# saninsteinn/django-assistant-bot

Measured on AMD Instinct MI355X. Metric: RAG queries/sec + p50 end-to-end latency, bge-base + Llama-3-8B, 1/2/4/8 MI355X, higher is better.
Workload: dtype bf16; 1 GPU; model=bge-base-en + llama-3-8b, global_batch=128, seq_len=1090, parallelism=dp1, mode=batch, index_rows=1000000, index=single shard, local top-k (no collective), sampling=temperature=1.0 top_k=50 top_p=0.95 ignore_eos, graphs=True

## Files before the change

### django_assistant_bot_amd/csrc/bindings.cpp

```cpp
#include <hip/hip_runtime.h>
#include <pybind11/numpy.h>
#include <pybind11/pybind11.h>
#include <pybind11/stl.h>

#include <stdexcept>
#include <string>

#include "kernels/launchers.h"
#include "runtime/json_grammar.h"
#include "runtime/kv_manager.h"
#include "runtime/rag.h"
#include "runtime/tokenizer.h"
#include "runtime/trace.h"

namespace py = pybind11;
using u = uintptr_t;

#define VP(x) reinterpret_cast<void*>(x)
#define CVP(x) reinterpret_cast<const void*>(x)
#define ST(x) reinterpret_cast<hipStream_t>(x)

static void check(int err, const char* name) {
  if (err) throw std::runtime_error(std::string("dab kernel '") + name + "' failed: " + hipGetErrorString((hipError_t)err));
}
// ... 91 lines not shown
                                     (const int*)ctx_k, batch, max_sq, Hq, Hkv, D, causal, paged, scale, ST(s)),
                "flash_attention");
        });
  m.def("flash_attention_rope",
        [](u q, long qst, long qsh, u kc, u vc, u bt, int max_blocks, int bs, u out, long ost, long osh, u cu_q,
           u ctx_k, int batch, int max_sq, int Hq, int Hkv, int D, int causal, float scale, u rope_pos, u rope_cs,
           u s) {
          check(dab::flash_attention(CVP(q), qst, qsh, nullptr, nullptr, 0, 0, CVP(kc), CVP(vc), (const int*)bt,
                                     max_blocks, bs, VP(out), ost, osh, (const int*)cu_q, nullptr, (const int*)ctx_k,
                                     batch, max_sq, Hq, Hkv, D, causal, 1, scale, ST(s), (const int*)rope_pos,
                                     CVP(rope_cs)),
                "flash_attention_rope");
        });
  m.def("create_cu_masked_stream", [](std::vector<uint32_t> mask) {
    hipStream_t st = nullptr;
    check(hipExtStreamCreateWithCUMask(&st, (uint32_t)mask.size(), mask.data()), "hipExtStreamCreateWithCUMask");
    return reinterpret_cast<uintptr_t>(st);
  });
  m.def("destroy_stream", [](u s) { check(hipStreamDestroy(ST(s)), "hipStreamDestroy"); });
  m.def("paged_decode_attention", [](u q, u kc, u vc, u bt, int max_blocks, int bs, u ctx, u out, u po, u pm, u pl,
                                     u cnt, int batch, int Hq, int Hkv, int D, int part_size, int max_parts,
                                     float scale, u s, u order, u w0, long w0_bytes, u w1, long w1_bytes,
                                     int w_blocks) {
    dab::L3Warm warm{{(const char*)w0, (const char*)w1}, {w0_bytes, w1_bytes}, w_blocks};
    check(dab::paged_decode_attention(CVP(q), CVP(kc), CVP(vc), (const int*)bt, max_blocks, bs, (const int*)ctx, VP(out),
                                      (float*)po, (float*)pm, (float*)pl, (int*)cnt, batch, Hq, Hkv, D, part_size,
                                      max_parts, scale, ST(s), (const int*)order, &warm),
          "paged_decode_attention");
  }, py::arg("q"), py::arg("kc"), py::arg("vc"), py::arg("bt"), py::arg("max_blocks"), py::arg("bs"), py::arg("ctx"),
     py::arg("out"), py::arg("po"), py::arg("pm"), py::arg("pl"), py::arg("cnt"), py::arg("batch"), py::arg("Hq"),
     py::arg("Hkv"), py::arg("D"), py::arg("part_size"), py::arg("max_parts"), py::arg("scale"), py::arg("s"),
     py::arg("order") = 0, py::arg("w0") = 0, py::arg("w0_bytes") = 0, py::arg("w1") = 0, py::arg("w1_bytes") = 0,
     py::arg("w_blocks") = 0);
  m.def("rope_kv_write_fp8", [](u qkv, int ld, u positions, u cos_sin, u q_out, u k_data, u k_exp, u v_data, u v_exp,
                                u slots, int T, int Hq, int Hkv, int D, int block_size, u s, u slabs, int S,
                                long slab_stride, int slab_bf16) {
    check(dab::rope_kv_write_fp8(CVP(qkv), ld, (const int*)positions, CVP(cos_sin), VP(q_out), VP(k_data), VP(k_exp),
                                 VP(v_data), VP(v_exp), (const int64_t*)slots, T, Hq, Hkv, D, block_size, ST(s),
                                 CVP(slabs), S, slab_stride, slab_bf16),
          "rope_kv_write_fp8");
  }, py::arg("qkv"), py::arg("ld"), py::arg("positions"), py::arg("cos_sin"), py::arg("q_out"), py::arg("k_data"),
     py::arg("k_exp"), py::arg("v_data"), py::arg("v_exp"), py::arg("slots"), py::arg("T"), py::arg("Hq"),
     py::arg("Hkv"), py::arg("D"), py::arg("block_size"), py::arg("s"), py::arg("slabs") = 0, py::arg("S") = 0,
     py::arg("slab_stride") = 0, py::arg("slab_bf16") = 0);
  m.def("kv_fp8_dequant_blocks", [](u k_data, u k_exp, u v_data, u v_exp, u ids, int n, u k_out, u v_out, int Hkv,
                                    int block_size, int D, u s) {
    check(dab::kv_fp8_dequant_blocks(CVP(k_data), CVP(k_exp), CVP(v_data), CVP(v_exp), (const int*)ids, n, VP(k_out),
                                     VP(v_out), Hkv, block_size, D, ST(s)),
          "kv_fp8_dequant_blocks");
  });
  m.def("paged_decode_attention_fp8", [](u q, u k_data, u k_exp, u v_data, u v_exp, u bt, int max_blocks, int bs, u ctx,
                                         u out, u po, u pm, u pl, u cnt, int batch, int Hq, int Hkv, int D,
                                         int part_size, int max_parts, float scale, u s, u order) {
    check(dab::paged_decode_attention_fp8(CVP(q), CVP(k_data), CVP(k_exp), CVP(v_data), CVP(v_exp), (const int*)bt,
                                          max_blocks, bs, (const int*)ctx, VP(out), (float*)po, (float*)pm, (float*)pl,
                                          (int*)cnt, batch, Hq, Hkv, D, part_size, max_parts, scale, ST(s),
                                          (const int*)order),
          "paged_decode_attention_fp8");
  });
  m.def("gemm_bt", [](u A, long lda, u B, long ldb, u C, long ldc, u bias, u residual, long ldr, int M, int N, int K,
                      int epilogue, int out_f32, u row_group, u q_group, u allow, int allow_words, u s, int b_rows,
                      int b_group) {
    check(dab::gemm_bt(CVP(A), lda, CVP(B), ldb, VP(C), ldc, CVP(bias), CVP(residual), ldr, M, N, K, epilogue, out_f32,
                       (const int*)row_group, (const int*)q_group, (const uint32_t*)allow, allow_words, ST(s), b_rows,
                       b_group),
          "gemm_bt");
// ... 291 lines not shown
```

### django_assistant_bot_amd/csrc/kernels/attention.hip

```cpp
#include <cstdlib>

#include "common.h"
#include "launchers.h"

#include <type_traits>

#define DAB_ALWAYS_INLINE __attribute__((always_inline))

namespace dab {

constexpr float kNegInf = -__builtin_huge_valf();

template <int D>
__device__ __forceinline__ int swz(int r, int c) {
  constexpr int RB = D * 2;
  constexpr int CPR = D / 8;
  constexpr int RPB = (256 / RB) > 0 ? (256 / RB) : 1;
  return r * RB + 16 * (c ^ ((2 * (r / RPB)) & (CPR - 1)));
}

struct FlashParams {
  const bf16* q;
  long q_stride_tok, q_stride_head;
  const bf16* k;
// ... 1246 lines not shown
        for (int t = 0; t < NTD; ++t) o[t] = f32x4{0.f, 0.f, 0.f, 0.f};
        m_run = -1e30f;
        l_run = 0.f;
      }
    }
    if (n.it < 0) break;
    if (new_q) {
#pragma unroll
      for (int kk = 0; kk < NKK; ++kk) qf[kk] = qn[kk];
    }
    c = n;
  }
}


struct DecodeParams {
  const bf16* q;
  const bf16* k_cache;
  const bf16* v_cache;
  const int* block_tables;
  int max_blocks, block_size;
  const int* ctx_lens;
  bf16* out;
  float* part_o;
  float* part_m;
  float* part_l;
  int* counters;
  const int* order;
  int Hq, Hkv, part_size, max_parts;
  float scale_log2;
  L3Warm warm;
};

template <int D, bool KV_NT, bool DMA = false, int NSLOT = 1>
__global__ __launch_bounds__(256, NSLOT == 1 ? 2 : 1) void paged_decode_kernel(DecodeParams p, int total_items) {
  static_assert(NSLOT == 1 || (NSLOT == 2 && DMA), "two slots: DMA staging only");
  const int attn_blocks = gridDim.x - p.warm.blocks;
  if ((int)blockIdx.x >= attn_blocks) {
    l3_warm(p.warm, blockIdx.x - attn_blocks);
    return;
  }
  constexpr int KT = 32;
  constexpr int NKK = D / 32;
  constexpr int NTD = D / 16;
  constexpr int CPR = D / 8;
  constexpr int SUB_BYTES = KT * D * 2;
  constexpr int CH = KT * CPR / 64;
  constexpr int RED_BYTES = 4 * 16 * D * 4 + 2 * 4 * 16 * 4;
  constexpr int STAGE_BYTES = 4 * 2 * SUB_BYTES * NSLOT;
  constexpr int AREA_BYTES = STAGE_BYTES > RED_BYTES + 16 ? STAGE_BYTES : RED_BYTES + 16;
  __shared__ __attribute__((aligned(16))) char smem[AREA_BYTES];
  int* last_flag = reinterpret_cast<int*>(smem + RED_BYTES);

  const int G = p.Hq / p.Hkv;
  const int tid = threadIdx.x, lane = tid & 63, g = lane >> 4, li = lane & 15;
  const int w = __builtin_amdgcn_readfirstlane(tid >> 6);
  char* ks = smem + w * 2 * SUB_BYTES * NSLOT;
  char* vs = ks + SUB_BYTES;

  const int BH = total_items / p.max_parts;
  int maxc = 0;
  for (int i = lane; i < BH / p.Hkv; i += 64) maxc = max(maxc, p.ctx_lens[i]);
#pragma unroll
  for (int off = 32; off; off >>= 1) maxc = max(maxc, __shfl_xor(maxc, off));
  maxc = __builtin_amdgcn_readfirstlane(maxc);
  const int live_items = min(p.max_parts, (maxc + p.part_size - 1) / p.part_size) * BH;
  for (int item = blockIdx.x; item < live_items; item += attn_blocks) {
    const int part = item / BH;
    const int bh = item - part * BH;
    const int hk = bh % p.Hkv, b = p.order ? p.order[bh / p.Hkv] : bh / p.Hkv;
    const int ctx = p.ctx_lens[b];
    const int k_begin = part * p.part_size;
    if (k_begin >= ctx) continue;
    const int k_end = min(ctx, k_begin + p.part_size);

    bf16x8 qf[NKK];
    {
      const bool qv = li < G;
      const bf16* qrow = p.q + ((size_t)b * p.Hq + hk * G + (qv ? li : 0)) * D;
#pragma unroll
      for (int kk = 0; kk < NKK; ++kk) {
        bf16x8 z = {0, 0, 0, 0, 0, 0, 0, 0};
        qf[kk] = qv ? *reinterpret_cast<const bf16x8*>(qrow + 32 * kk + 8 * g) : z;
      }
    }

    u32x4 kA[CH], vA[CH], kB[CH], vB[CH];
    const int k_last = ((k_end - 1) / KT) * KT;
    auto load_sub = [&](u32x4(&kr)[CH], u32x4(&vr)[CH], int k0) {
      const int kc = min(k0, k_last);
      const int blk = p.block_tables[(size_t)b * p.max_blocks + kc / p.block_size];
      const size_t base = (((size_t)blk * p.Hkv + hk) * p.block_size + (kc % p.block_size)) * D;
      const int bytes = k0 > k_last ? 0 : min(KT, k_end - k0) * D * 2;
      const auto kd = __builtin_amdgcn_make_buffer_rsrc((void*)(p.k_cache + base), 0, bytes, 0x00020000);
      const auto vd = __builtin_amdgcn_make_buffer_rsrc((void*)(p.v_cache + base), 0, bytes, 0x00020000);
#pragma unroll
      for (int c = 0; c < CH; ++c) {
        kr[c] = __builtin_bit_cast(u32x4, __builtin_amdgcn_raw_buffer_load_b128(kd, lane * 16, c * 1024, KV_NT ? 2 : 0));
        vr[c] = __builtin_bit_cast(u32x4, __builtin_amdgcn_raw_buffer_load_b128(vd, lane * 16, c * 1024, KV_NT ? 2 : 0));
      }
    };
    auto stage = [&](const u32x4(&kr)[CH], const u32x4(&vr)[CH]) {
#pragma unroll
      for (int c = 0; c < CH; ++c) {
        const int idx = lane + c * 64;
        const int row = idx / CPR, ch = idx % CPR;
        *reinterpret_cast<u32x4*>(ks + swz<D>(row, ch)) = kr[c];
        *reinterpret_cast<u32x4*>(vs + swz<D>(row, ch)) = vr[c];
      }
    };

    f32x4 o[NTD];
#pragma unroll
    for (int t = 0; t < NTD; ++t) o[t] = f32x4{0.f, 0.f, 0.f, 0.f};
    float m_run = -1e30f, l_run = 0.f;

    auto compute = [&](const int k0) {
      __builtin_amdgcn_s_waitcnt(0xc07f);
// ... 36 lines not shown
      }
      l_run = l_run * alpha + ls;
      m_run = m_new;
      bf16x8 pb;
#pragma unroll
      for (int j = 0; j < 4; ++j) {
        pb[j] = (short)f2bf(s[0][j]);
        pb[j + 4] = (short)f2bf(s[1][j]);
      }
      const int qq = li >> 2, pp = li & 3;
#pragma unroll
      for (int t = 0; t < NTD; ++t) {
        o[t] *= alpha;
        const int ch = 2 * t + (pp >> 1);
        const int boff = 8 * (pp & 1);
        const bf16x4 lo = ds_read_tr16(vs + swz<D>(4 * g + qq, ch) + boff);
        const bf16x4 hi = ds_read_tr16(vs + swz<D>(16 + 4 * g + qq, ch) + boff);
        const bf16x8 a = {lo[0], lo[1], lo[2], lo[3], hi[0], hi[1], hi[2], hi[3]};
        o[t] = mfma16(a, pb, o[t]);
      }
      __builtin_amdgcn_s_waitcnt(0xc07f);
      __builtin_amdgcn_wave_barrier();
    };
    const int kw = k_begin + w * KT;
    if constexpr (DMA) {
      static_assert(D == 128, "DMA staging assumes 256-B rows (4 rows per 1 KB piece)");
      const int drow = lane >> 4;
      auto blk_at = [&](int k0) {
        return p.block_tables[(size_t)b * p.max_blocks + min(k0, k_last) / p.block_size];
      };
      auto dma = [&](int k0, int blk) {
        const int kc = min(k0, k_last);
        const size_t base = (((size_t)blk * p.Hkv + hk) * p.block_size + (kc % p.block_size)) * D;
        const int bytes = k0 > k_last ? 0 : min(KT, k_end - k0) * D * 2;
        const auto kd = __builtin_amdgcn_make_buffer_rsrc((void*)(p.k_cache + base), 0, bytes, 0x00020000);
        const auto vd = __builtin_amdgcn_make_buffer_rsrc((void*)(p.v_cache + base), 0, bytes, 0x00020000);
#pragma unroll
        for (int i = 0; i < KT / 4; ++i) {
          const int row = 4 * i + drow;
          const unsigned off = (unsigned)(row * 256 + 16 * ((lane & 15) ^ ((2 * row) & 15)));
          __builtin_amdgcn_raw_ptr_buffer_load_lds(kd, (__attribute__((address_space(3))) void*)(ks + i * 1024), 16, off,
                                                   0, 0, KV_NT ? 2 : 0);
          __builtin_amdgcn_raw_ptr_buffer_load_lds(vd, (__attribute__((address_space(3))) void*)(vs + i * 1024), 16, off,
                                                   0, 0, KV_NT ? 2 : 0);
        }
      };
      if constexpr (NSLOT == 2) {
        char* const slot0 = smem + w * 2 * SUB_BYTES * NSLOT;
        const int n_sub = kw < k_end ? (k_end - kw + 4 * KT - 1) / (4 * KT) : 0;
        const int myblk = lane < n_sub ? blk_at(kw + lane * 4 * KT) : 0;
        auto issue = [&](int i) {
          ks = slot0 + (i & 1) * 2 * SUB_BYTES;
          vs = ks + SUB_BYTES;
          dma(kw + i * 4 * KT, __builtin_amdgcn_readlane(myblk, i));
        };
        if (n_sub > 0) issue(0);
        for (int i = 0; i < n_sub; ++i) {
          if (i + 1 < n_sub) {
            issue(i + 1);
            asm volatile("s_waitcnt vmcnt(16)" ::: "memory");
          } else {
            asm volatile("s_waitcnt vmcnt(0)" ::: "memory");
          }
          ks = slot0 + (i & 1) * 2 * SUB_BYTES;
          vs = ks + SUB_BYTES;
          compute(kw + i * 4 * KT);
        }
      } else {
      int blk = __builtin_amdgcn_readfirstlane(blk_at(kw));
      for (int k0 = kw; k0 < k_end; k0 += 4 * KT) {
        dma(k0, blk);
        blk = blk_at(k0 + 4 * KT);
        asm volatile("s_waitcnt vmcnt(1)" ::: "memory");
        compute(k0);
        blk = __builtin_amdgcn_readfirstlane(blk);
      }
      asm volatile("s_waitcnt vmcnt(0)" ::: "memory");
      }
    } else {
      load_sub(kA, vA, kw);
      load_sub(kB, vB, kw + 4 * KT);
      for (int k0 = kw; k0 < k_end; k0 += 8 * KT) {
        stage(kA, vA);
        load_sub(kA, vA, k0 + 8 * KT);
        compute(k0);
        if (k0 + 4 * KT >= k_end) break;
        stage(kB, vB);
        load_sub(kB, vB, k0 + 12 * KT);
        compute(k0 + 4 * KT);
      }
    }

    l_run += __shfl_xor(l_run, 16, 64);
    l_run += __shfl_xor(l_run, 32, 64);
    __syncthreads();
    float* ored = reinterpret_cast<float*>(smem);
    float* mred = ored + 4 * 16 * D;
    float* lred = mred + 4 * 16;
#pragma unroll
    for (int t = 0; t < NTD; ++t) *reinterpret_cast<f32x4*>(ored + (w * 16 + li) * D + 16 * t + 4 * g) = o[t];
    if (g == 0) {
      mred[w * 16 + li] = m_run;
      lred[w * 16 + li] = l_run;
    }
    __syncthreads();
    const int np = min(p.max_parts, div_up(ctx, p.part_size));
    const bool direct = np == 1;
// ... 157 lines not shown
  dim3 grid((max_seqlen_q + qb - 1) / qb, Hq, batch);
#define DAB_FLASH(DD, C, P)                                                                          \
  do {                                                                                              \
    if (wide)                                                                                       \
      hipLaunchKernelGGL((flash_fwd_kernel<DD, C, P, (DD == 128 ? 8 : 4), 1>), grid,              \
                         dim3(DD == 128 ? 512 : 256), 0, s, prm);                                   \
    else if (DD == 64 && enc5)                                                                      \
      hipLaunchKernelGGL((flash_fwd_kernel<DD, C, P, 4, 1, DD == 64 ? 5 : 0>), grid, dim3(256), 0, s, prm); \
    else                                                                                            \
      hipLaunchKernelGGL((flash_fwd_kernel<DD, C, P, 4, 1>), grid, dim3(256), 0, s, prm);           \
  } while (0)
#define DAB_FLASH_D(DD)                    \
  if (paged) {                             \
    if (causal) DAB_FLASH(DD, true, true); \
    else DAB_FLASH(DD, false, true);       \
  } else {                                 \
    if (causal) DAB_FLASH(DD, true, false); \
    else DAB_FLASH(DD, false, false);      \
  }
  if (D == 128) {
    DAB_FLASH_D(128)
  } else if (D == 64) {
    DAB_FLASH_D(64)
  } else if (D == 32) {
    DAB_FLASH_D(32)
  } else {
    return hipErrorInvalidValue;
  }
#undef DAB_FLASH_D
#undef DAB_FLASH
  return hipGetLastError();
}

int paged_decode_attention(const void* q, const void* k_cache, const void* v_cache, const int* block_tables,
                           int max_blocks, int block_size, const int* ctx_lens, void* out, float* part_o,
                           float* part_m, float* part_l, int* counters, int batch, int Hq, int Hkv, int D,
                           int part_size, int max_parts, float scale, hipStream_t s, const int* order,
                           const L3Warm* warm) {
  if (batch <= 0) return 0;
  if (Hq % Hkv || Hq / Hkv > 16 || part_size % 128 || max_parts < 1 || block_size % 32) return hipErrorInvalidValue;
  if (max_parts > 1 && !counters) return hipErrorInvalidValue;
  if (!q) return hipErrorInvalidValue;
  DecodeParams prm;
  prm.q = (const bf16*)q;
  prm.k_cache = (const bf16*)k_cache;
  prm.v_cache = (const bf16*)v_cache;
  prm.block_tables = block_tables;
  prm.max_blocks = max_blocks;
  prm.block_size = block_size;
  prm.ctx_lens = ctx_lens;
  prm.out = (bf16*)out;
  prm.part_o = part_o;
  prm.part_m = part_m;
  prm.part_l = part_l;
  prm.counters = counters;
  prm.order = order;
  prm.Hq = Hq;
  prm.Hkv = Hkv;
  prm.part_size = part_size;
  prm.max_parts = max_parts;
  prm.scale_log2 = scale * 1.4426950408889634f;
  prm.warm = warm ? *warm : L3Warm{{nullptr, nullptr}, {0, 0}, 0};
  if (prm.warm.blocks < 0 || prm.warm.blocks > 1024 || ((prm.warm.bytes[0] | prm.warm.bytes[1]) & 15) ||
      (prm.warm.blocks && prm.warm.bytes[0] + prm.warm.bytes[1] <= 0))
    return hipErrorInvalidValue;
  const int total_items = max_parts * Hkv * batch;
  dim3 grid((total_items < 2048 ? total_items : 2048) + prm.warm.blocks);
  if (D == 128) {
    if (batch * Hkv <= 64 && part_size <= 64 * 4 * 32)
      hipLaunchKernelGGL((paged_decode_kernel<128, true, true, 2>), grid, dim3(256), 0, s, prm, total_items);
    else hipLaunchKernelGGL((paged_decode_kernel<128, true, true>), grid, dim3(256), 0, s, prm, total_items);
  } else if (D == 64) {
    hipLaunchKernelGGL((paged_decode_kernel<64, true>), grid, dim3(256), 0, s, prm, total_items);
  } else {
    return hipErrorInvalidValue;
  }
  return hipGetLastError();
}

}
```

### django_assistant_bot_amd/csrc/kernels/launchers.h

```cpp
#pragma once
#include <hip/hip_runtime.h>
#include <stddef.h>
#include <stdint.h>

#include <string>
#include <vector>

namespace dab {

inline int div_up_host(int a, int b) { return (a + b - 1) / b; }

struct L3Warm {
  const char* ptr[2];
  long bytes[2];
  int blocks;
};

int rmsnorm(void* out, void* res_out, const void* x, const void* res_in, const void* w, int rows, int cols, float eps,
            hipStream_t s);
int rmsnorm_slabs(void* out, void* res_out, const void* slabs, int S, long slab_stride, const void* res_in,
                  const void* w, int rows, int cols, float eps, hipStream_t s, int slab_bf16 = 0);
int layernorm(void* out, const void* x, const void* res_in, const void* gamma, const void* beta, int rows, int cols,
              float eps, hipStream_t s);
int bert_embed(void* out, const int* ids, const int* pos_ids, const int* type_ids, const void* word, const void* pos,
               const void* type, const void* gamma, const void* beta, int rows, int cols, float eps, hipStream_t s);
int embed_gather(void* out, const int* ids, const void* table, int rows, int cols, hipStream_t s);
int mean_pool(float* out, void* out_bf16, const void* hidden, const int* cu_seqlens, int batch, int cols,
              int normalize, hipStream_t s);

int gelu(void* out, const void* x, const void* bias, size_t rows, int cols, hipStream_t s);
int silu_mul(void* out, const void* x, size_t rows, int F, hipStream_t s, int interleaved = 0);
int rope_kv_write(const void* qkv, int ld, const int* positions, const void* cos_sin, void* q_out, void* k_cache,
                  void* v_cache, const int64_t* slots, int T, int Hq, int Hkv, int D, int block_size, hipStream_t s,
                  const void* slabs = nullptr, int S = 0, long slab_stride = 0, int slab_bf16 = 0);

int flash_attention(const void* q, long q_stride_tok, long q_stride_head, const void* k, const void* v,
                    long kv_stride_tok, long kv_stride_head, const void* k_cache, const void* v_cache,
                    const int* block_tables, int max_blocks, int block_size, void* out, long o_stride_tok,
                    long o_stride_head, const int* cu_q, const int* cu_k, const int* ctx_k, int batch,
                    int max_seqlen_q, int Hq, int Hkv, int D, int causal, int paged, float scale, hipStream_t s,
                    const int* rope_pos = nullptr, const void* rope_cs = nullptr);
int paged_decode_attention(const void* q, const void* k_cache, const void* v_cache, const int* block_tables,
                           int max_blocks, int block_size, const int* ctx_lens, void* out, float* part_o,
                           float* part_m, float* part_l, int* counters, int batch, int Hq, int Hkv, int D,
                           int part_size, int max_parts, float scale, hipStream_t s,
                           const int* order = nullptr, const L3Warm* warm = nullptr);

int rope_kv_write_fp8(const void* qkv, int ld, const int* positions, const void* cos_sin, void* q_out, void* k_data,
                      void* k_exp, void* v_data, void* v_exp, const int64_t* slots, int T, int Hq, int Hkv, int D,
                      int block_size, hipStream_t s, const void* slabs = nullptr, int S = 0, long slab_stride = 0,
                      int slab_bf16 = 0);
int kv_fp8_dequant_blocks(const void* k_data, const void* k_exp, const void* v_data, const void* v_exp,
                          const int* block_ids, int n, void* k_out, void* v_out, int Hkv, int block_size, int D,
                          hipStream_t s);
int paged_decode_attention_fp8(const void* q, const void* k_data, const void* k_exp, const void* v_data,
                               const void* v_exp, const int* block_tables, int max_blocks, int block_size,
                               const int* ctx_lens, void* out, float* part_o, float* part_m, float* part_l,
                               int* counters, int batch, int Hq, int Hkv, int D, int part_size, int max_parts,
                               float scale, hipStream_t s, const int* order = nullptr);

int gemm_bt(const void* A, long lda, const void* B, long ldb, void* C, long ldc, const void* bias, const void* residual,
            long ldr, int M, int N, int K, int epilogue, int out_f32, const int* row_group, const int* q_group,
            const uint32_t* allow, int allow_words, hipStream_t s, int b_rows = 0, int b_group = 1);

int gemm256_ok(int M, int N, int K, long lda, long ldb);
int gemm256_candidates(const void* A, long lda, const void* B, long ldb, int M, int N, int K, const int* row_group,
                       const int* q_group, const float* thr, int* cnt, float* cand_val, int* cand_idx, int cap,
                       hipStream_t s, int b_rows = 0);
int gemm256_candidates_stamped(const void* A, long lda, const void* B, int M, int N, int K, int b_rows,
                               const float* thr, int* cnt, float* cand_val, int* cand_idx, int cap, void* stamps,
                               int stamp_tiles, hipStream_t s);
int gemm256_stamped(const void* A, long lda, const void* B, void* C, const void* bias, const void* residual, int M,
                    int N, int K, int epilogue, int b_shuf, void* stamps, int stamp_tiles, hipStream_t s, int store_aux);
int gemm256(const void* A, long lda, const void* B, long ldb, void* C, long ldc, const void* bias,
            const void* residual, long ldr, int M, int N, int K, int epilogue, hipStream_t s, int b_shuf = 0,
            int b_group = 1, const int* rows = nullptr, int src_rows = 0);

int gemm_mid_ok(int M, int N, int K, long lda);
long gemm_mid_slab_bytes();
// ... 76 lines not shown
```

### django_assistant_bot_amd/models/llama.py

```python
from __future__ import annotations

from dataclasses import dataclass

import torch

from .. import ops
from ..ops import reference as ref
from .configs import DecoderConfig


@dataclass
class DecoderLayer:

    attn_norm: torch.Tensor
    qkv_w: torch.Tensor
    o_w: torch.Tensor
    mlp_norm: torch.Tensor
    gate_up_w: torch.Tensor
    down_w: torch.Tensor


class Fp8Proj:

    __slots__ = ("w", "data", "exps", "group")
# ... 68 lines not shown
        if dev.type == "cuda" and head_dim != 128:
            raise ValueError("the FP8 KV cache kernels take head_dim 128 only")
        self.k = torch.zeros((layers, num_blocks, kv_heads, block_size, head_dim), device=dev, dtype=torch.uint8)
        self.v = torch.zeros_like(self.k)
        self.k_exp = torch.full((layers, num_blocks, kv_heads, block_size), 127, device=dev, dtype=torch.uint8)
        self.v_exp = torch.full_like(self.k_exp, 127)
        if dev.type == "cuda":
            self.scratch_blocks = max(1, int(scratch_blocks) or num_blocks)
            self.scratch_k = torch.zeros((self.scratch_blocks, kv_heads, block_size, head_dim), device=dev, dtype=dtype)
            self.scratch_v = torch.zeros_like(self.scratch_k)

    @staticmethod
    def bytes_per_block(layers, kv_heads, block_size, head_dim, dtype=torch.bfloat16, kv_dtype: str = "bf16"):
        if kv_dtype == "fp8":
            return 2 * layers * kv_heads * block_size * (head_dim + 1)
        return 2 * layers * kv_heads * block_size * head_dim * torch.finfo(dtype).bits // 8

    @staticmethod
    def scratch_bytes(scratch_blocks, kv_heads, block_size, head_dim, dtype=torch.bfloat16):
        return 2 * scratch_blocks * kv_heads * block_size * head_dim * torch.finfo(dtype).bits // 8

    def write(self, li, qkv, positions, cos_sin, slots, Hq, Hkv, D, write_q=True):
        if self.fp8:
            return ops.rope_kv_write_fp8(qkv, positions, cos_sin, self.k[li], self.k_exp[li], self.v[li], self.v_exp[li],
                                         slots, Hq, Hkv, D, write_q=write_q)
        return ops.rope_kv_write(qkv, positions, cos_sin, self.k[li], self.v[li], slots, Hq, Hkv, D, write_q=write_q)

    def decode_attention(self, li, q, block_tables, ctx_lens, part_size, workspace, out=None, order=None, warm=None):
        if self.fp8:
            return ops.paged_decode_fp8(q, self.k[li], self.k_exp[li], self.v[li], self.v_exp[li], block_tables, ctx_lens,
                                        part_size, workspace, out=out, order=order, warm=warm)
        return ops.paged_decode(q, self.k[li], self.v[li], block_tables, ctx_lens, part_size, workspace, out=out,
                                order=order, warm=warm)

    def prefill_attention(self, li, q, meta, out=None, rope=None):
        if not self.fp8:
            return ops.flash_attention_paged(q, self.k[li], self.v[li], meta.block_tables, meta.cu_q, meta.ctx_lens,
                                             meta.max_q, causal=True, out=out, rope=rope)
        plan = None
        if q.is_cuda:
            if meta.kv_groups is None:
                p = ops.kv_prefill_plan(meta.block_tables, meta.ctx_lens, meta.cu_q, self.block_size,
                                        self.scratch_blocks, q.device)
                meta.kv_blocks, meta.kv_scratch_bt, meta.kv_groups = p.blocks, p.scratch_bt, p.groups
            plan = ops.KVPrefillPlan(meta.kv_blocks, meta.kv_scratch_bt, meta.kv_groups)
        return ops.flash_attention_paged_fp8(q, self.k[li], self.k_exp[li], self.v[li], self.v_exp[li], meta.block_tables,
                                             meta.cu_q, meta.ctx_lens, meta.max_q, causal=True, out=out, rope=rope,
                                             scratch=(self.scratch_k, self.scratch_v), plan=plan)


class LlamaModel:
    VOCAB_PAD = 384

    def __init__(self, cfg: DecoderConfig, weights: dict, device, tp_group=None, tp_size: int = 1,
                 interleaved_mlp: bool = False, fragment_layout: bool = True, consume: bool = False,
                 tp_rank: int | None = None, vocab_parallel: bool = True, small_norm_fused: bool | None = None,
                 weight_dtype: str = "bf16"):
        if weight_dtype not in ("bf16", "fp8"):
            raise ValueError(f"weight_dtype must be 'bf16' or 'fp8', got {weight_dtype!r}")
        if weight_dtype == "fp8" and tp_size > 1:
            raise ValueError("weight_dtype='fp8' is not supported under tensor parallelism (tp_size > 1)")
        self.weight_dtype = weight_dtype
        self.cfg = cfg
        self.device = torch.device(device)
        if tp_rank is None:
            tp_rank = 0
# ... 132 lines not shown
        elif M <= 16 and N % nat.stream_gemm_bn(self.STREAM_CFG_M16) == 0:
            cfg = self.STREAM_CFG_M16
        elif M <= 32 and N % nat.stream_gemm_bn(self.STREAM_CFG_M32) == 0:
            cfg = self.STREAM_CFG_M32
        elif M <= 64:
            cfg = self.STREAM_CFG_M64
        else:
            cfg = self.STREAM_WIDE.get(name)
            if cfg is None or N % nat.stream_gemm_bn(cfg):
                cfg = self.STREAM_CFG_M128
        return cfg if N % nat.stream_gemm_bn(cfg) == 0 else -1

    @staticmethod
    def _stream_splits(N: int, K: int, bn: int = 128) -> int:
        tiles, best = N // bn, 1
        for s in (1, 2, 4, 8, 16):
            if K % (128 * s):
                break
            best = s
            if tiles * s >= 192:
                break
        return best

    def _stream_choice(self, name: str, M: int, N: int, K: int) -> tuple[int, int]:
        cfg = self._stream_cfg(name, M, N)
        if cfg < 0 or K % 128:
            return -1, 1
        return cfg, self._stream_splits(N, K, ops.native().stream_gemm_bn(cfg))

    PROJ_GROUPS = {"gate_up": 8}

    slab_bf16 = True

    fp8_qkv_slab_f32 = True

    def _proj(self, x, w, dec: bool, allow_slabs: bool = True, name: str = "", epilogue=ops.EPI_NONE,
              slab_f32: bool = False):
        if not x.is_cuda:
            if epilogue == ops.EPI_SWIGLU8 or (epilogue == ops.EPI_NONE and name == "gate_up"):
                y = ops.linear(x, w)
                return ops.silu_mul(y, group=8 if self.interleaved_mlp else 0)
            return ops.linear(x, w)
        grp = self.proj_group.get(name, 1)
        if dec and self.frag:
            cfg, s = self._stream_choice(name, x.shape[0], w.shape[0], w.shape[1])
            if cfg >= 0:
                sw, e = self._stream_w(w, name, cfg)
                if epilogue != ops.EPI_NONE:
                    return ops.stream_gemm(x, sw, epilogue=epilogue, nt=True, cfg=cfg, w_group=grp, w_exps=e)
                sd = torch.bfloat16 if (self.slab_bf16 and self.tp_size == 1 and not slab_f32) else torch.float32
                out = ops.stream_gemm(x, sw, splits=s, cfg=cfg, nt=True, slab_dtype=sd, w_group=grp, w_exps=e)
                return ops.slab_reduce(out) if (s > 1 and not allow_slabs) else out
        return ops.gemm_bt(x, _bf16_copy(w), epilogue=epilogue, shuffled=self.frag, b_group=grp)

    FP8_STREAM_OFF: frozenset = frozenset()
    fp8_stream = True

    def _stream_w(self, w, name: str, cfg: int):
        if not isinstance(w, Fp8Proj):
            return w, None
        if self.fp8_stream and ops.native().stream_gemm_fp8_ok(cfg) and (name, cfg) not in self.FP8_STREAM_OFF:
            return w.data, w.exps
        return w.w, None

    prune_last_tail = True

# ... 82 lines not shown
            return self.custom_ar.all_reduce_rmsnorm(x.t, residual, w, self.cfg.eps)
        return ops.rmsnorm(x, w, self.cfg.eps, residual=residual)

    tp_fused_norm = True

    def _tp_partial(self, x, cols: int):
        ar = self.custom_ar
        if self.tp_fused_norm and ar is not None and x.is_cuda and ar.norm_eligible(x, cols):
            return _Partial(x)
        if x.dtype == torch.float32 and x.dim() == 3:
            x = ops.slab_reduce(x)
        return self._all_reduce(x)

    def _layer(self, li: int, L: DecoderLayer, x, residual, meta: AttnMeta, kv: KVCache, sk: bool, rows=None):
        cfg, D, T = self.cfg, self.cfg.head_dim, meta.positions.numel()
        slabs_ok = self.tp_size == 1
        fuse = not sk and self.tp_size == 1 and (x if x is not None else residual).is_cuda
        if x is None:
            h, _ = ops.rmsnorm(residual, L.attn_norm, cfg.eps)
        elif residual is None:
            h, _ = ops.rmsnorm(x, L.attn_norm, cfg.eps)
            residual = x
        else:
            h, residual = self._norm(x, L.attn_norm, residual)
        qkv = self._proj(h, L.qkv_w, sk, name="qkv", slab_f32=kv.fp8 and self.fp8_qkv_slab_f32)
        if (not meta.decode and not meta.n_decode and qkv.is_cuda and qkv.dtype == torch.bfloat16 and qkv.dim() == 2
                and ops.kernels.flash_rope_ok(D, kv.block_size)):
            kv.write(li, qkv, meta.positions, self.cos_sin, meta.slots, self.hq, self.hkv, D, write_q=False)
            q = qkv[:, :self.hq * D].view(T, self.hq, D)
            a = kv.prefill_attention(li, q, meta, rope=(meta.positions, self.cos_sin))
            if rows is not None:
                return self._layer_tail_rows(L, a, residual, rows, T, D)
            return self._layer_tail(L, a, residual, sk, fuse, slabs_ok, T, D)
        q = kv.write(li, qkv, meta.positions, self.cos_sin, meta.slots, self.hq, self.hkv, D)
        if meta.decode:
            a = kv.decode_attention(li, q, meta.block_tables, meta.ctx_lens, meta.part_size, meta.workspace,
                                    order=meta.order, warm=self._warm(L, T, q))
        elif meta.n_decode:
            a = self._mixed_attention(q, kv, li, meta)
        else:
            a = kv.prefill_attention(li, q, meta)
        if rows is not None:
            return self._layer_tail_rows(L, a, residual, rows, T, D)
        return self._layer_tail(L, a, residual, sk, fuse, slabs_ok, T, D)

    def _layer_tail_rows(self, L, a, residual, rows, T, D):
        n = rows.numel()
        if n == 0:
            return None, residual.new_empty((0, residual.shape[1]))
        if rows.dtype != torch.int32:
            rows = rows.to(torch.int32)
        pg = self.proj_group
        res = ops.gemm_bt(a.view(T, self.hq * D), _bf16_copy(L.o_w), residual=residual, shuffled=True,
                          b_group=pg.get("o", 1), rows=rows)
        h, _ = ops.rmsnorm(res, L.mlp_norm, self.cfg.eps)
        act = ops.gemm_bt(h, _bf16_copy(L.gate_up_w), epilogue=ops.EPI_SWIGLU8, shuffled=True,
                          b_group=pg.get("gate_up", 1), as_m=T)
        return None, ops.gemm_bt(act, _bf16_copy(L.down_w), residual=res, shuffled=True, b_group=pg.get("down", 1),
                                 as_m=T)

    def _layer_tail(self, L, a, residual, sk, fuse, slabs_ok, T, D):
        cfg = self.cfg
        if fuse:
            residual = ops.gemm_bt(a.view(T, self.hq * D), _bf16_copy(L.o_w), residual=residual, shuffled=self.frag,
                                   b_group=self.proj_group.get("o", 1))
            h, _ = ops.rmsnorm(residual, L.mlp_norm, cfg.eps)
# ... 40 lines not shown
```

### django_assistant_bot_amd/ops/__init__.py

```python
from ._lib import has_native, native
from .kernels import (
    EPI_GELU,
    EPI_NONE,
    EPI_SCORES,
    EPI_SWIGLU,
    EPI_SWIGLU8,
    DecodeWorkspace,
    KVPrefillPlan,
    flash_attention_paged_fp8,
    kv_dequant_blocks,
    kv_dequantize,
    kv_prefill_plan,
    kv_quantize,
    paged_decode_fp8,
    rope_kv_write_fp8,
    bert_embed,
    embed_gather,
    flash_attention_packed,
    flash_attention_paged,
    gelu,
    gemm_bt,
    interleave_gate_up,
    regroup_gate_up,
    slab_reduce,
    shuffle_weights,
    unshuffle_weights,
    shuffle_weights_fp8,
    unshuffle_weights_fp8,
    weight_dequantize_fp8,
    weight_quantize_fp8,
    stream_gemm,
    score_candidates,
    score_candidates_shuffled,
    shuffle_rows_into,
    STREAM_MAX_M,
    layernorm,
    linear,
    mean_pool,
    paged_decode,
    rmsnorm,
    rope_kv_write,
    mask_logits,
    sample_candidates,
    sample_merge,
    sample_tokens,
    silu_mul,
    topk_rows,
)
```

### django_assistant_bot_amd/ops/kernels.py

```python
from __future__ import annotations

import math

import torch
import torch.nn.functional as F

from . import reference as ref
from ._lib import expect, expect_bf16_contig, native, ptr, same_device, stream

EPI_NONE, EPI_GELU, EPI_SWIGLU, EPI_SCORES = ref.EPI_NONE, ref.EPI_GELU, ref.EPI_SWIGLU, ref.EPI_SCORES
EPI_SWIGLU8 = ref.EPI_SWIGLU8


def _i32(t: torch.Tensor) -> None:
    if t.dtype != torch.int32 or not t.is_contiguous():
        raise TypeError("expected a contiguous int32 tensor")




def rmsnorm(x: torch.Tensor, w: torch.Tensor, eps: float, residual: torch.Tensor | None = None):
    slabs = x.dim() == 3 and x.dtype in (torch.float32, torch.bfloat16)
    if not x.is_cuda:
        if slabs:
# ... 231 lines not shown
        return ref.paged_decode(q, k_cache, v_cache, block_tables, ctx_lens, scale)
    _i32(ctx_lens)
    _i32(block_tables)
    expect_bf16_contig(q, k_cache, v_cache)
    Hkv, bs = k_cache.shape[1], k_cache.shape[2]
    expect(D in (64, 128), "decode head dim must be 64 or 128")
    expect(Hq % Hkv == 0 and Hq // Hkv <= 16, "GQA group must be <= 16")
    expect(part_size % 128 == 0, "part_size must be a multiple of 128")
    expect(block_tables.shape[0] >= B and ctx_lens.numel() >= B, "block table / ctx_lens rows < batch")
    max_parts = workspace.max_parts if workspace is not None else 1
    if workspace is None:
        part_size = max(part_size, ((block_tables.shape[1] * bs + 127) // 128) * 128)
        ws_o = ws_m = ws_l = ws_c = None
    else:
        expect(workspace.o.numel() >= B * Hq * max_parts * D and workspace.cnt.numel() >= B * Hkv,
               "decode workspace too small")
        ws_o, ws_m, ws_l, ws_c = workspace.o, workspace.m, workspace.l, workspace.cnt
    out = torch.empty_like(q) if out is None else out
    if order is not None:
        _i32(order)
        expect(order.is_cuda and order.numel() >= B, "decode order must hold the batch")
    wargs = {}
    if warm is not None and warm[1] > 0:
        ranges, blocks = warm
        expect(1 <= len(ranges) <= 2 and 0 < blocks <= 1024, "warm: 1-2 ranges, 1-1024 workgroups")
        for i, (t, nb) in enumerate(ranges):
            expect(t.is_cuda and t.is_contiguous() and 0 < nb <= t.numel() * t.element_size() and nb % 16 == 0,
                   "warm range must be a 16-B multiple inside a contiguous device tensor")
            wargs[f"w{i}"], wargs[f"w{i}_bytes"] = ptr(t), int(nb)
        wargs["w_blocks"] = int(blocks)
    native().paged_decode_attention(ptr(q), ptr(k_cache), ptr(v_cache), ptr(block_tables), block_tables.shape[1], bs,
                                    ptr(ctx_lens), ptr(out), ptr(ws_o), ptr(ws_m), ptr(ws_l), ptr(ws_c), B, Hq, Hkv,
                                    D, int(part_size), int(max_parts), float(scale), stream(q), ptr(order), **wargs)
    return out



kv_quantize = ref.kv_quantize
kv_dequantize = ref.kv_dequantize


def _expect_fp8_cache(k_data, k_exp, v_data, v_exp):
    for t in (k_data, k_exp, v_data, v_exp):
        if t.dtype != torch.uint8 or not t.is_contiguous():
            raise TypeError("the FP8 KV cache is contiguous uint8 (data and exponent bytes)")
    same_device(k_data, k_exp, v_data, v_exp)
    expect(k_data.dim() == 4 and k_data.shape == v_data.shape and tuple(k_exp.shape) == tuple(k_data.shape[:3])
           and k_exp.shape == v_exp.shape, "FP8 cache: data [blocks, Hkv, block_size, D], exponents [blocks, Hkv, block_size]")
    expect(k_data.shape[3] == 128, "the FP8 KV cache kernels take head dim 128 only")


def rope_kv_write_fp8(qkv, positions, cos_sin, k_data, k_exp, v_data, v_exp, slots, Hq, Hkv, D, write_q=True):
    block_size = k_data.shape[2]
    slabs = qkv.dim() == 3 and qkv.dtype in (torch.float32, torch.bfloat16)
    if not qkv.is_cuda:
        if slabs:
            qkv = qkv.float().sum(0).to(torch.bfloat16)
        q = ref.rope_kv_write_fp8(qkv, positions, cos_sin, k_data, k_exp, v_data, v_exp, slots, Hq, Hkv, D, block_size)
        return q if write_q else None
    expect(D == 128, "the FP8 KV cache kernels take head dim 128 only")
    _expect_fp8_cache(k_data, k_exp, v_data, v_exp)
    _i32(positions)
    expect(slots.dtype == torch.int64 and slots.is_contiguous(), "slots must be contiguous int64")
    expect(cos_sin.dtype == torch.float32 and cos_sin.is_contiguous(), "cos_sin must be contiguous fp32")
    T = qkv.shape[-2]
    expect(qkv.shape[-1] == (Hq + 2 * Hkv) * D, "qkv width mismatch")
# ... 686 lines not shown
```

Before: 40.32 queries/s.

## Fuse RoPE and KV-cache write into the paged decode attention kernel

Adds a fused decode path that applies RoPE to Q/K straight from the QKV projection output (plain or split-K slabs), writes the new K/V token into the paged cache, and patches it into the staged shared-memory tile. The attention loads then skip the newest token. This removes the separate rope_kv_write launch per layer and its round trip of Q through global memory during decode. In exchange the kernel has more shared memory, an extra barrier and more template variants, and every work item recomputes the Q RoPE for its partition.

```diff
diff --git a/django_assistant_bot_amd/csrc/bindings.cpp b/django_assistant_bot_amd/csrc/bindings.cpp
--- a/django_assistant_bot_amd/csrc/bindings.cpp
+++ b/django_assistant_bot_amd/csrc/bindings.cpp
@@ -147,6 +147,22 @@
      py::arg("Hkv"), py::arg("D"), py::arg("part_size"), py::arg("max_parts"), py::arg("scale"), py::arg("s"),
      py::arg("order") = 0, py::arg("w0") = 0, py::arg("w0_bytes") = 0, py::arg("w1") = 0, py::arg("w1_bytes") = 0,
      py::arg("w_blocks") = 0);
+  m.def("paged_decode_rope", [](u qkv, int ld, u slabs, int S, long slab_stride, int slab_bf16, u positions, u cos_sin,
+                                u slots, u kc, u vc, u bt, int max_blocks, int bs, u ctx, u out, u po, u pm, u pl, u cnt,
+                                int batch, int Hq, int Hkv, int D, int part_size, int max_parts, float scale, u s,
+                                u order, u w0, long w0_bytes, u w1, long w1_bytes, int w_blocks) {
+    dab::L3Warm warm{{(const char*)w0, (const char*)w1}, {w0_bytes, w1_bytes}, w_blocks};
+    check(dab::paged_decode_rope(CVP(qkv), ld, CVP(slabs), S, slab_stride, slab_bf16, (const int*)positions,
+                                 CVP(cos_sin), (const int64_t*)slots, VP(kc), VP(vc), (const int*)bt, max_blocks, bs,
+                                 (const int*)ctx, VP(out), (float*)po, (float*)pm, (float*)pl, (int*)cnt, batch, Hq, Hkv,
+                                 D, part_size, max_parts, scale, ST(s), (const int*)order, &warm),
+          "paged_decode_rope");
+  }, py::arg("qkv"), py::arg("ld"), py::arg("slabs"), py::arg("S"), py::arg("slab_stride"), py::arg("slab_bf16"),
+     py::arg("positions"), py::arg("cos_sin"), py::arg("slots"), py::arg("kc"), py::arg("vc"), py::arg("bt"),
+     py::arg("max_blocks"), py::arg("bs"), py::arg("ctx"), py::arg("out"), py::arg("po"), py::arg("pm"), py::arg("pl"),
+     py::arg("cnt"), py::arg("batch"), py::arg("Hq"), py::arg("Hkv"), py::arg("D"), py::arg("part_size"),
+     py::arg("max_parts"), py::arg("scale"), py::arg("s"), py::arg("order") = 0, py::arg("w0") = 0,
+     py::arg("w0_bytes") = 0, py::arg("w1") = 0, py::arg("w1_bytes") = 0, py::arg("w_blocks") = 0);
   m.def("rope_kv_write_fp8", [](u qkv, int ld, u positions, u cos_sin, u q_out, u k_data, u k_exp, u v_data, u v_exp,
                                 u slots, int T, int Hq, int Hkv, int D, int block_size, u s, u slabs, int S,
                                 long slab_stride, int slab_bf16) {
diff --git a/django_assistant_bot_amd/csrc/kernels/attention.hip b/django_assistant_bot_amd/csrc/kernels/attention.hip
--- a/django_assistant_bot_amd/csrc/kernels/attention.hip
+++ b/django_assistant_bot_amd/csrc/kernels/attention.hip
@@ -1302,9 +1302,21 @@
   L3Warm warm;
 };
 
-template <int D, bool KV_NT, bool DMA = false, int NSLOT = 1>
-__global__ __launch_bounds__(256, NSLOT == 1 ? 2 : 1) void paged_decode_kernel(DecodeParams p, int total_items) {
+struct DecodeRope {
+  const void* src;
+  long slab_stride;
+  int S, ld, plain;
+  const int* positions;
+  const float2* cos_sin;
+  const int64_t* slots;
+};
+
+template <int D, bool KV_NT, bool DMA = false, int NSLOT = 1, typename RT = void>
+__global__ __launch_bounds__(256, NSLOT == 1 ? 2 : 1) void paged_decode_kernel(DecodeParams p, int total_items,
+                                                                                DecodeRope rp) {
   static_assert(NSLOT == 1 || (NSLOT == 2 && DMA), "two slots: DMA staging only");
+  constexpr bool ROPE = !std::is_void<RT>::value;
+  static_assert(!ROPE || (DMA && D == 128), "fused RoPE prologue: the D = 128 DMA kernel only");
   const int attn_blocks = gridDim.x - p.warm.blocks;
   if ((int)blockIdx.x >= attn_blocks) {
     l3_warm(p.warm, blockIdx.x - attn_blocks);
@@ -1319,8 +1331,10 @@
   constexpr int RED_BYTES = 4 * 16 * D * 4 + 2 * 4 * 16 * 4;
   constexpr int STAGE_BYTES = 4 * 2 * SUB_BYTES * NSLOT;
   constexpr int AREA_BYTES = STAGE_BYTES > RED_BYTES + 16 ? STAGE_BYTES : RED_BYTES + 16;
-  __shared__ __attribute__((aligned(16))) char smem[AREA_BYTES];
+  constexpr int ROPE_BYTES = ROPE ? 18 * D * 2 : 0;
+  __shared__ __attribute__((aligned(16))) char smem[AREA_BYTES + ROPE_BYTES];
   int* last_flag = reinterpret_cast<int*>(smem + RED_BYTES);
+  char* const qs = smem + AREA_BYTES;
 
   const int G = p.Hq / p.Hkv;
   const int tid = threadIdx.x, lane = tid & 63, g = lane >> 4, li = lane & 15;
@@ -1345,7 +1359,7 @@
     const int k_end = min(ctx, k_begin + p.part_size);
 
     bf16x8 qf[NKK];
-    {
+    if constexpr (!ROPE) {
       const bool qv = li < G;
       const bf16* qrow = p.q + ((size_t)b * p.Hq + hk * G + (qv ? li : 0)) * D;
 #pragma unroll
@@ -1354,6 +1368,73 @@
         qf[kk] = qv ? *reinterpret_cast<const bf16x8*>(qrow + 32 * kk + 8 * g) : z;
       }
     }
+    bool own = false;
+    int64_t slot = -1;
+    int pos = 0;
+    if constexpr (ROPE) {
+      slot = rp.slots[b];
+      pos = rp.positions[b];
+      own = slot >= 0 && k_end == ctx;
+    }
+    const int k_new = ctx - 1;
+    const int k_ld = own ? k_end - 1 : k_end;
+    u32x4 nv1 = {0, 0, 0, 0}, nv2 = {0, 0, 0, 0};
+    auto rope_tasks = [&]() DAB_ALWAYS_INLINE {
+      if constexpr (ROPE) {
+        const int nq = 8 * G;
+        if (tid < nq + 16) {
+          const int c = tid & 7, row = tid >> 3;
+          const bool is_v = row == G + 1;
+          const int h = row < G ? hk * G + row : (is_v ? p.Hq + p.Hkv + hk : p.Hq + hk);
+          float2 cs[8];
+          rope_cs(rp.cos_sin, pos, D / 2, 8 * c, cs);
+          float x1[8], x2[8];
+          constexpr int U = sizeof(RT) == 4 ? 2 : 4;
+          rope_chunk<U, RT>(rp.plain ? (const bf16*)rp.src : nullptr, rp.plain ? nullptr : (const RT*)rp.src, rp.S,
+                            rp.slab_stride, rp.ld, b, h, D, 8 * c, cs, !is_v, x1, x2);
+          nv1 = pack8(x1);
+          nv2 = pack8(x2);
+          *reinterpret_cast<u32x4*>(qs + row * (D * 2) + 16 * c) = nv1;
+          *reinterpret_cast<u32x4*>(qs + row * (D * 2) + D + 16 * c) = nv2;
+        }
+      }
+    };
+    auto rope_store = [&]() DAB_ALWAYS_INLINE {
+      if constexpr (ROPE) {
+        const int row = tid >> 3;
+        if (own && row >= G && row < G + 2) {
+          const int64_t blk = (slot >> 32) ? slot / p.block_size : (int64_t)((uint32_t)slot / (uint32_t)p.block_size);
+          const int64_t off = slot - blk * p.block_size;
+          bf16* dst = const_cast<bf16*>(row == G + 1 ? p.v_cache : p.k_cache) +
+                      (((size_t)blk * p.Hkv + hk) * p.block_size + off) * D + 8 * (tid & 7);
+          *reinterpret_cast<u32x4*>(dst) = nv1;
+          *reinterpret_cast<u32x4*>(dst + D / 2) = nv2;
+        }
+      }
+    };
+    auto rope_sync_q = [&]() DAB_ALWAYS_INLINE {
+      if constexpr (ROPE) {
+        asm volatile("s_waitcnt lgkmcnt(0)" ::: "memory");
+        __builtin_amdgcn_s_barrier();
+        asm volatile("" ::: "memory");
+        const bool qv = li < G;
+#pragma unroll
+        for (int kk = 0; kk < NKK; ++kk) {
+          bf16x8 z = {0, 0, 0, 0, 0, 0, 0, 0};
+          qf[kk] = qv ? *reinterpret_cast<const bf16x8*>(qs + (qv ? li : 0) * (D * 2) + (32 * kk + 8 * g) * 2) : z;
+        }
+      }
+    };
+    const bool own_w = ROPE && own && w == (((k_new - k_begin) / KT) & 3);
+    auto rope_patch = [&](const int k0) DAB_ALWAYS_INLINE {
+      if constexpr (ROPE) {
+        if (own_w && k_new - k0 < KT && lane < 2 * CPR) {
+          const int isv = lane / CPR, ch = lane % CPR;
+          const u32x4 v = *reinterpret_cast<const u32x4*>(qs + (G + isv) * (D * 2) + 16 * ch);
+          *reinterpret_cast<u32x4*>((isv ? vs : ks) + swz<D>(k_new - k0, ch)) = v;
+        }
+      }
+    };
 
     u32x4 kA[CH], vA[CH], kB[CH], vB[CH];
     const int k_last = ((k_end - 1) / KT) * KT;
@@ -1456,7 +1537,7 @@
       auto dma = [&](int k0, int blk) {
         const int kc = min(k0, k_last);
         const size_t base = (((size_t)blk * p.Hkv + hk) * p.block_size + (kc % p.block_size)) * D;
-        const int bytes = k0 > k_last ? 0 : min(KT, k_end - k0) * D * 2;
+        const int bytes = k0 > k_last ? 0 : min(KT, k_ld - k0) * D * 2;
         const auto kd = __builtin_amdgcn_make_buffer_rsrc((void*)(p.k_cache + base), 0, bytes, 0x00020000);
         const auto vd = __builtin_amdgcn_make_buffer_rsrc((void*)(p.v_cache + base), 0, bytes, 0x00020000);
 #pragma unroll
@@ -1478,7 +1559,10 @@
           vs = ks + SUB_BYTES;
           dma(kw + i * 4 * KT, __builtin_amdgcn_readlane(myblk, i));
         };
+        rope_tasks();
         if (n_sub > 0) issue(0);
+        rope_store();
+        rope_sync_q();
         for (int i = 0; i < n_sub; ++i) {
           if (i + 1 < n_sub) {
             issue(i + 1);
@@ -1488,15 +1572,25 @@
           }
           ks = slot0 + (i & 1) * 2 * SUB_BYTES;
           vs = ks + SUB_BYTES;
+          rope_patch(kw + i * 4 * KT);
           compute(kw + i * 4 * KT);
         }
       } else {
-      int blk = __builtin_amdgcn_readfirstlane(blk_at(kw));
+      int blk = blk_at(kw);
+      rope_tasks();
+      blk = __builtin_amdgcn_readfirstlane(blk);
+      if constexpr (ROPE) {
+        if (kw < k_end) dma(kw, blk);
+        rope_store();
+        rope_sync_q();
+      }
       for (int k0 = kw; k0 < k_end; k0 += 4 * KT) {
-        dma(k0, blk);
+        if (!ROPE || k0 != kw) dma(k0, blk);
         blk = blk_at(k0 + 4 * KT);
         asm volatile("s_waitcnt vmcnt(1)" ::: "memory");
+        rope_patch(k0);
         compute(k0);
+        if constexpr (ROPE) __builtin_amdgcn_sched_barrier(0);
         blk = __builtin_amdgcn_readfirstlane(blk);
       }
       asm volatile("s_waitcnt vmcnt(0)" ::: "memory");
@@ -1720,15 +1814,15 @@
   return hipGetLastError();
 }
 
-int paged_decode_attention(const void* q, const void* k_cache, const void* v_cache, const int* block_tables,
-                           int max_blocks, int block_size, const int* ctx_lens, void* out, float* part_o,
-                           float* part_m, float* part_l, int* counters, int batch, int Hq, int Hkv, int D,
-                           int part_size, int max_parts, float scale, hipStream_t s, const int* order,
-                           const L3Warm* warm) {
+static int launch_paged_decode(const void* q, const void* k_cache, const void* v_cache, const int* block_tables,
+                               int max_blocks, int block_size, const int* ctx_lens, void* out, float* part_o,
+                               float* part_m, float* part_l, int* counters, int batch, int Hq, int Hkv, int D,
+                               int part_size, int max_parts, float scale, hipStream_t s, const int* order,
+                               const L3Warm* warm, const DecodeRope* rope, int slab_bf16) {
   if (batch <= 0) return 0;
   if (Hq % Hkv || Hq / Hkv > 16 || part_size % 128 || max_parts < 1 || block_size % 32) return hipErrorInvalidValue;
   if (max_parts > 1 && !counters) return hipErrorInvalidValue;
-  if (!q) return hipErrorInvalidValue;
+  if (!q && !rope) return hipErrorInvalidValue;
   DecodeParams prm;
   prm.q = (const bf16*)q;
   prm.k_cache = (const bf16*)k_cache;
@@ -1754,16 +1848,63 @@
     return hipErrorInvalidValue;
   const int total_items = max_parts * Hkv * batch;
   dim3 grid((total_items < 2048 ? total_items : 2048) + prm.warm.blocks);
+  const bool two_slots = batch * Hkv <= 64 && part_size <= 64 * 4 * 32;
+  if (rope) {
+    if (D != 128) return hipErrorInvalidValue;
+    const bool b16 = slab_bf16 && !rope->plain;
+    if (two_slots && b16)
+      hipLaunchKernelGGL((paged_decode_kernel<128, true, true, 2, bf16>), grid, dim3(256), 0, s, prm, total_items, *rope);
+    else if (two_slots)
+      hipLaunchKernelGGL((paged_decode_kernel<128, true, true, 2, float>), grid, dim3(256), 0, s, prm, total_items, *rope);
+    else if (b16)
+      hipLaunchKernelGGL((paged_decode_kernel<128, true, true, 1, bf16>), grid, dim3(256), 0, s, prm, total_items, *rope);
+    else
+      hipLaunchKernelGGL((paged_decode_kernel<128, true, true, 1, float>), grid, dim3(256), 0, s, prm, total_items, *rope);
+    return hipGetLastError();
+  }
+  const DecodeRope none{};
   if (D == 128) {
-    if (batch * Hkv <= 64 && part_size <= 64 * 4 * 32)
-      hipLaunchKernelGGL((paged_decode_kernel<128, true, true, 2>), grid, dim3(256), 0, s, prm, total_items);
-    else hipLaunchKernelGGL((paged_decode_kernel<128, true, true>), grid, dim3(256), 0, s, prm, total_items);
+    if (two_slots)
+      hipLaunchKernelGGL((paged_decode_kernel<128, true, true, 2>), grid, dim3(256), 0, s, prm, total_items, none);
+    else hipLaunchKernelGGL((paged_decode_kernel<128, true, true>), grid, dim3(256), 0, s, prm, total_items, none);
   } else if (D == 64) {
-    hipLaunchKernelGGL((paged_decode_kernel<64, true>), grid, dim3(256), 0, s, prm, total_items);
+    hipLaunchKernelGGL((paged_decode_kernel<64, true>), grid, dim3(256), 0, s, prm, total_items, none);
   } else {
     return hipErrorInvalidValue;
   }
   return hipGetLastError();
 }
 
+int paged_decode_attention(const void* q, const void* k_cache, const void* v_cache, const int* block_tables,
+                           int max_blocks, int block_size, const int* ctx_lens, void* out, float* part_o,
+                           float* part_m, float* part_l, int* counters, int batch, int Hq, int Hkv, int D,
+                           int part_size, int max_parts, float scale, hipStream_t s, const int* order,
+                           const L3Warm* warm) {
+  return launch_paged_decode(q, k_cache, v_cache, block_tables, max_blocks, block_size, ctx_lens, out, part_o, part_m,
+                             part_l, counters, batch, Hq, Hkv, D, part_size, max_parts, scale, s, order, warm, nullptr,
+                             0);
 }
+
+int paged_decode_rope(const void* qkv, int ld, const void* slabs, int S, long slab_stride, int slab_bf16,
+                      const int* positions, const void* cos_sin, const int64_t* slots, void* k_cache, void* v_cache,
+                      const int* block_tables, int max_blocks, int block_size, const int* ctx_lens, void* out,
+                      float* part_o, float* part_m, float* part_l, int* counters, int batch, int Hq, int Hkv, int D,
+                      int part_size, int max_parts, float scale, hipStream_t s, const int* order, const L3Warm* warm) {
+  if (!positions || !cos_sin || !slots || (!qkv && !slabs) || ld % 8 || ld < (Hq + 2 * Hkv) * D)
+    return hipErrorInvalidValue;
+  if (slabs && (S < 1 || slab_stride % 8)) return hipErrorInvalidValue;
+  DecodeRope rp{};
+  rp.src = slabs ? slabs : qkv;
+  rp.plain = slabs ? 0 : 1;
+  rp.S = slabs ? S : 1;
+  rp.slab_stride = slab_stride;
+  rp.ld = ld;
+  rp.positions = positions;
+  rp.cos_sin = (const float2*)cos_sin;
+  rp.slots = slots;
+  return launch_paged_decode(nullptr, k_cache, v_cache, block_tables, max_blocks, block_size, ctx_lens, out, part_o,
+                             part_m, part_l, counters, batch, Hq, Hkv, D, part_size, max_parts, scale, s, order, warm,
+                             &rp, slab_bf16);
+}
+
+}
diff --git a/django_assistant_bot_amd/csrc/kernels/launchers.h b/django_assistant_bot_amd/csrc/kernels/launchers.h
--- a/django_assistant_bot_amd/csrc/kernels/launchers.h
+++ b/django_assistant_bot_amd/csrc/kernels/launchers.h
@@ -45,6 +45,12 @@
                            float* part_m, float* part_l, int* counters, int batch, int Hq, int Hkv, int D,
                            int part_size, int max_parts, float scale, hipStream_t s,
                            const int* order = nullptr, const L3Warm* warm = nullptr);
+int paged_decode_rope(const void* qkv, int ld, const void* slabs, int S, long slab_stride, int slab_bf16,
+                      const int* positions, const void* cos_sin, const int64_t* slots, void* k_cache, void* v_cache,
+                      const int* block_tables, int max_blocks, int block_size, const int* ctx_lens, void* out,
+                      float* part_o, float* part_m, float* part_l, int* counters, int batch, int Hq, int Hkv, int D,
+                      int part_size, int max_parts, float scale, hipStream_t s, const int* order = nullptr,
+                      const L3Warm* warm = nullptr);
 
 int rope_kv_write_fp8(const void* qkv, int ld, const int* positions, const void* cos_sin, void* q_out, void* k_data,
                       void* k_exp, void* v_data, void* v_exp, const int64_t* slots, int T, int Hq, int Hkv, int D,
diff --git a/django_assistant_bot_amd/models/llama.py b/django_assistant_bot_amd/models/llama.py
--- a/django_assistant_bot_amd/models/llama.py
+++ b/django_assistant_bot_amd/models/llama.py
@@ -124,6 +124,11 @@
                                         part_size, workspace, out=out, order=order, warm=warm)
         return ops.paged_decode(q, self.k[li], self.v[li], block_tables, ctx_lens, part_size, workspace, out=out,
                                 order=order, warm=warm)
+
+    def write_decode_attention(self, li, qkv, positions, cos_sin, slots, Hq, Hkv, D, block_tables, ctx_lens, part_size,
+                               workspace, order=None, warm=None):
+        return ops.paged_decode_rope(qkv, positions, cos_sin, slots, self.k[li], self.v[li], block_tables, ctx_lens,
+                                     Hq, Hkv, D, part_size, workspace, order=order, warm=warm)
 
     def prefill_attention(self, li, q, meta, out=None, rope=None):
         if not self.fp8:
@@ -322,6 +327,8 @@
 
     slab_bf16 = True
 
+    fused_decode_rope = True
+
     fp8_qkv_slab_f32 = True
 
     def _proj(self, x, w, dec: bool, allow_slabs: bool = True, name: str = "", epilogue=ops.EPI_NONE,
@@ -470,6 +477,11 @@
             if rows is not None:
                 return self._layer_tail_rows(L, a, residual, rows, T, D)
             return self._layer_tail(L, a, residual, sk, fuse, slabs_ok, T, D)
+        if meta.decode and self.fused_decode_rope and not kv.fp8:
+            a = kv.write_decode_attention(li, qkv, meta.positions, self.cos_sin, meta.slots, self.hq, self.hkv, D,
+                                          meta.block_tables, meta.ctx_lens, meta.part_size, meta.workspace,
+                                          order=meta.order, warm=self._warm(L, T, qkv))
+            return self._layer_tail(L, a, residual, sk, fuse, slabs_ok, T, D)
         q = kv.write(li, qkv, meta.positions, self.cos_sin, meta.slots, self.hq, self.hkv, D)
         if meta.decode:
             a = kv.decode_attention(li, q, meta.block_tables, meta.ctx_lens, meta.part_size, meta.workspace,
diff --git a/django_assistant_bot_amd/ops/__init__.py b/django_assistant_bot_amd/ops/__init__.py
--- a/django_assistant_bot_amd/ops/__init__.py
+++ b/django_assistant_bot_amd/ops/__init__.py
@@ -38,6 +38,7 @@
     linear,
     mean_pool,
     paged_decode,
+    paged_decode_rope,
     rmsnorm,
     rope_kv_write,
     mask_logits,
diff --git a/django_assistant_bot_amd/ops/kernels.py b/django_assistant_bot_amd/ops/kernels.py
--- a/django_assistant_bot_amd/ops/kernels.py
+++ b/django_assistant_bot_amd/ops/kernels.py
@@ -287,6 +287,69 @@
     native().paged_decode_attention(ptr(q), ptr(k_cache), ptr(v_cache), ptr(block_tables), block_tables.shape[1], bs,
                                     ptr(ctx_lens), ptr(out), ptr(ws_o), ptr(ws_m), ptr(ws_l), ptr(ws_c), B, Hq, Hkv,
                                     D, int(part_size), int(max_parts), float(scale), stream(q), ptr(order), **wargs)
+    return out
+
+
+def paged_decode_rope(qkv, positions, cos_sin, slots, k_cache, v_cache, block_tables, ctx_lens, Hq, Hkv, D,
+                      part_size=512, workspace: DecodeWorkspace | None = None, scale=None, out=None, order=None,
+                      warm=None):
+    scale = 1.0 / math.sqrt(D) if scale is None else scale
+    slabs = qkv.dim() == 3 and qkv.dtype in (torch.float32, torch.bfloat16)
+    B = qkv.shape[-2]
+    if not qkv.is_cuda or D != 128:
+        q = rope_kv_write(qkv, positions, cos_sin, k_cache, v_cache, slots, Hq, Hkv, D)
+        return paged_decode(q, k_cache, v_cache, block_tables, ctx_lens, part_size, workspace, scale=scale, out=out,
+                            order=order, warm=warm)
+    expect_bf16_contig(k_cache, v_cache)
+    same_device(qkv, positions, cos_sin, slots, k_cache, v_cache, block_tables, ctx_lens)
+    _i32(positions)
+    _i32(ctx_lens)
+    _i32(block_tables)
+    expect(slots.dtype == torch.int64 and slots.is_contiguous(), "slots must be contiguous int64")
+    expect(cos_sin.dtype == torch.float32 and cos_sin.is_contiguous(), "cos_sin must be contiguous fp32")
+    expect(qkv.shape[-1] == (Hq + 2 * Hkv) * D, "qkv width mismatch")
+    expect(positions.numel() == B and slots.numel() == B, "positions / slots length mismatch")
+    bs = k_cache.shape[2]
+    expect(tuple(k_cache.shape[1:]) == (Hkv, bs, D) and k_cache.shape == v_cache.shape, "cache shape mismatch")
+    expect(cos_sin.shape[1] == D // 2, "cos/sin table width mismatch")
+    expect(Hq % Hkv == 0 and Hq // Hkv <= 16, "GQA group must be <= 16")
+    expect(part_size % 128 == 0, "part_size must be a multiple of 128")
+    expect(block_tables.shape[0] >= B and ctx_lens.numel() >= B, "block table / ctx_lens rows < batch")
+    max_parts = workspace.max_parts if workspace is not None else 1
+    if workspace is None:
+        part_size = max(part_size, ((block_tables.shape[1] * bs + 127) // 128) * 128)
+        ws_o = ws_m = ws_l = ws_c = None
+    else:
+        expect(workspace.o.numel() >= B * Hq * max_parts * D and workspace.cnt.numel() >= B * Hkv,
+               "decode workspace too small")
+        ws_o, ws_m, ws_l, ws_c = workspace.o, workspace.m, workspace.l, workspace.cnt
+    if out is None:
+        out = torch.empty((B, Hq, D), dtype=torch.bfloat16, device=qkv.device)
+    expect(out.dtype == torch.bfloat16 and out.is_contiguous() and tuple(out.shape) == (B, Hq, D),
+           "out: contiguous bf16 [B, Hq, D]")
+    if order is not None:
+        _i32(order)
+        expect(order.is_cuda and order.numel() >= B, "decode order must hold the batch")
+    wargs = {}
+    if warm is not None and warm[1] > 0:
+        ranges, blocks = warm
+        expect(1 <= len(ranges) <= 2 and 0 < blocks <= 1024, "warm: 1-2 ranges, 1-1024 workgroups")
+        for i, (t, nb) in enumerate(ranges):
+            expect(t.is_cuda and t.is_contiguous() and 0 < nb <= t.numel() * t.element_size() and nb % 16 == 0,
+                   "warm range must be a 16-B multiple inside a contiguous device tensor")
+            wargs[f"w{i}"], wargs[f"w{i}_bytes"] = ptr(t), int(nb)
+        wargs["w_blocks"] = int(blocks)
+    if slabs:
+        expect(qkv.is_contiguous(), "slabs must be contiguous")
+        src = (0, qkv.shape[-1], ptr(qkv), qkv.shape[0], B * qkv.shape[-1], int(qkv.dtype == torch.bfloat16))
+    else:
+        expect(qkv.dim() == 2 and qkv.dtype == torch.bfloat16 and qkv.stride(1) == 1 and qkv.stride(0) % 8 == 0,
+               "qkv: bf16 rows with unit column stride")
+        src = (ptr(qkv), qkv.stride(0), 0, 0, 0, 0)
+    native().paged_decode_rope(*src, ptr(positions), ptr(cos_sin), ptr(slots), ptr(k_cache), ptr(v_cache),
+                               ptr(block_tables), block_tables.shape[1], bs, ptr(ctx_lens), ptr(out), ptr(ws_o),
+                               ptr(ws_m), ptr(ws_l), ptr(ws_c), B, Hq, Hkv, D, int(part_size), int(max_parts),
+                               float(scale), stream(qkv), ptr(order), **wargs)
     return out
 
 
```

Result: no change. 40.48 queries/s, median of 6 (+0.4%).
